# itxtx/normalizing-flows-study

Hardware: AMD Instinct MI355X
Metric: log_prob samples/sec/GPU + test-NLL match; RealNVP d=2 and MAF d=63 (higher is better)
Workload: dtype fp32

## Files before the change

normalizing-flows-study_amd/csrc/nfx_made.hip:

```cpp
#include "nfx_made_kernel.h"
#include "nfx_made_wide_kernel.h"
#include <atomic>
#include <cstdlib>

#include "nfx_made_seqs_kernel.h"
#include "nfx_pack.h"

namespace nfx {

__global__ void made_pack_kernel(NfxMlpRaw net, int d, int H, float* packed) {
    const int HT = (H + 31) / 32;
    const MadeLayout L = made_layout(d, HT);
    const int Hp = L.Hp, G1 = 4 * L.NKC;
    for (int i = blockIdx.x * blockDim.x + threadIdx.x; i < L.total; i += gridDim.x * blockDim.x) {
        if (i >= L.s_deg) continue;
        float v = 0.f;
        if (i < L.b1) {
            int t = i - L.w1, rr = t & 3, lane = (t >> 2) & 63, g = (t >> 8) % G1, ht = (t >> 8) / G1;
            int row = 32 * ht + (lane & 31), col = 2 * (4 * g + rr) + (lane >> 5);
            v = (row < H && col < d) ? mlp_weight(net, 0, d, row, col) : 0.f;
        } else if (i < L.w2) {
            int row = acc_vec_row(i - L.b1);
            v = row < H ? mlp_bias(net, 0, row) : 0.f;
        } else if (i < L.b2 || (i >= L.w3 && i < L.b3)) {
            const int layer = i < L.b2 ? 1 : 2;
            const ATileElem e = a_tile_elem(i - (layer == 1 ? L.w2 : L.w3));
            int row = 32 * (e.tile / HT) + e.row, col = 32 * (e.tile % HT) + e.k;
            v = (row < H && col < H) ? mlp_weight(net, layer, H, row, col) : 0.f;
        } else if (i < L.w3 || (i >= L.b3 && i < L.w4)) {
            const int layer = i < L.w3 ? 1 : 2;
            int row = acc_vec_row(i - (layer == 1 ? L.b2 : L.b3));
            v = row < H ? mlp_bias(net, layer, row) : 0.f;
        } else if (i < L.b4) {
            const ATileElem e = a_tile_elem(i - L.w4);
            int jw = e.tile / HT, which = jw & 1, j = jw >> 1;
            int orow = 32 * j + e.row, col = 32 * (e.tile % HT) + e.k;
            v = (orow < d && col < H) ? mlp_weight(net, 3, H, which * d + orow, col) : 0.f;
        } else if (i < L.par_total) {
            int t = i - L.b4, jw = t >> 5, which = jw & 1, j = jw >> 1;
            int orow = 32 * j + acc_vec_row(t & 31);
            v = orow < d ? mlp_bias(net, 3, which * d + orow) : 0.f;
        } else if (i < L.s_b1) {
            int t = i - L.s_w1t, ii = t / Hp, a = t % Hp;
            v = (ii < d && a < H) ? mlp_weight(net, 0, d, a, ii) : 0.f;
        } else if (i < L.s_w2) {
            int a = i - L.s_b1;
            v = a < H ? mlp_bias(net, 0, a) : 0.f;
        } else if (i < L.s_b2 || (i >= L.s_w3 && i < L.s_b3)) {
            const int layer = i < L.s_b2 ? 1 : 2;
            int t = i - (layer == 1 ? L.s_w2 : L.s_w3), a = t / Hp, b = t % Hp;
            v = (a < H && b < H) ? mlp_weight(net, layer, H, a, b) : 0.f;
        } else if (i < L.s_w3 || (i >= L.s_b3 && i < L.s_w4)) {
            const int layer = i < L.s_w3 ? 1 : 2;
            int a = i - (layer == 1 ? L.s_b2 : L.s_b3);
            v = a < H ? mlp_bias(net, layer, a) : 0.f;
        } else if (i < L.s_b4) {
            int t = i - L.s_w4, row = t / Hp, a = t % Hp;
            v = (row < 2 * d && a < H) ? mlp_weight(net, 3, H, row, a) : 0.f;
        } else if (i < L.s_deg) {
            int row = i - L.s_b4;
            v = row < 2 * d ? mlp_bias(net, 3, row) : 0.f;
        }
        packed[i] = v;
    }
}

constexpr int kLiveThreads = 1024;

__global__ __launch_bounds__(kLiveThreads) void made_live_kernel(NfxMlpRaw net, int d, int H, float* packed) {
    const int HT = (H + 31) / 32;
    const MadeLayout L = made_layout(d, HT);
    {
        __shared__ int deg[256];
        const int Hp = L.Hp;
        for (int a0 = 0; a0 < Hp; a0 += kLiveThreads / 16) {
            const int a = a0 + (threadIdx.x >> 4), q = threadIdx.x & 15;
            int n = 0;
            if (a < H && net.mask[0]) {
                const float* row = net.mask[0] + (size_t)a * d;
#pragma unroll 4
                for (int j = q; j < d; j += 16) n += row[j] != 0.f ? 1 : 0;
            }
            n += __shfl_xor(n, 1);
            n += __shfl_xor(n, 2);
            n += __shfl_xor(n, 4);
            n += __shfl_xor(n, 8);
            if (q == 0 && a < Hp) deg[a] = a < H ? (net.mask[0] ? n - 1 : 0) : 1000000000;
        }
        __syncthreads();
        for (int a = threadIdx.x; a < Hp; a += kLiveThreads) {
            const int da = deg[a];
            int rank = 0;
            for (int b = 0; b < Hp; ++b) rank += (deg[b] < da || (deg[b] == da && b < a)) ? 1 : 0;
            packed[L.s_deg + a] = (float)da;
            packed[L.s_deg + Hp + rank] = (float)da;
            packed[L.s_deg + 2 * Hp + rank] = (float)a;
        }
    }
    int* nk = reinterpret_cast<int*>(packed);
    for (int i = threadIdx.x; i < 3 * HT + L.NJ; i += kLiveThreads) nk[L.nk1 + i] = 0;
    __shared__ double red[256];
    const int rows[4] = {H, H, H, 2 * d}, cols[4] = {d, H, H, H};
    const double tsafe = block_mlp_tsafe(net, 4, rows, cols, 1.0e37, red);
    if (threadIdx.x == 0) packed[L.tsafe] = (float)fmin(tsafe, 3.0e38);
}

__global__ __launch_bounds__(256) void made_extent_kernel(int d, int H, float* packed) {
    const int HT = (H + 31) / 32;
    const MadeLayout L = made_layout(d, HT);
    int* nk = reinterpret_cast<int*>(packed);
    const int n1 = HT * 4 * L.NKC, n23 = HT * HT * 4, n4 = L.NJ * 2 * HT * 4;
    const int lane = lane_id();
    for (int gi = blockIdx.x * 4 + (threadIdx.x >> 6); gi < n1 + 2 * n23 + n4; gi += gridDim.x * 4) {
        int off, word, ext;
        if (gi < n1) {
            const int ht = gi / (4 * L.NKC), g = gi % (4 * L.NKC);
            off = L.w1 + gi * 256;
            word = L.nk1 + ht;
            ext = g / 4 + 1;
        } else if (gi < n1 + 2 * n23) {
            const int t = (gi - n1) % n23, layer = (gi - n1) / n23;
            off = (layer == 0 ? L.w2 : L.w3) + t * 256;
            word = (layer == 0 ? L.nk2 : L.nk3) + t / (HT * 4);
            ext = (t % (HT * 4)) / 4 + 1;
        } else {
            const int t = gi - n1 - 2 * n23;
            off = L.w4 + t * 256;
            word = L.nk4 + t / (2 * HT * 4);
            ext = (t % (HT * 4)) / 4 + 1;
        }
        const f32x4 v = *reinterpret_cast<const f32x4*>(packed + off + 4 * lane);
        const bool nzl = v[0] != 0.f || v[1] != 0.f || v[2] != 0.f || v[3] != 0.f;
        if (__ballot(nzl) != 0 && lane == 0) atomicMax(&nk[word], ext);
    }
}

template <int HT>
made_seqs_kernel_t made_seqs_pick_ht(int variant, bool logp) {
    if (variant == NFX_MAF_FORWARD) return made_seqs_kernel<HT, NFX_MAF_FORWARD, false>;
    return logp ? made_seqs_kernel<HT, NFX_IAF_INVERSE, true> : made_seqs_kernel<HT, NFX_IAF_INVERSE, false>;
}
template made_seqs_kernel_t made_seqs_pick_ht<1>(int, bool);
template made_seqs_kernel_t made_seqs_pick_ht<2>(int, bool);

template <int HT, int VAR>
static made_seq_kernel_t seq_var() {
    return made_seq_kernel<HT, VAR>;
}

template <int HT>
made_seq_kernel_t made_seq_pick_ht(int variant) {
    return variant == NFX_MAF_FORWARD ? seq_var<HT, NFX_MAF_FORWARD>() : seq_var<HT, NFX_IAF_INVERSE>();
}
template made_seq_kernel_t made_seq_pick_ht<1>(int);
template made_seq_kernel_t made_seq_pick_ht<2>(int);
template made_seq_kernel_t made_seq_pick_ht<3>(int);
template made_seq_kernel_t made_seq_pick_ht<4>(int);

static made_par_kernel_t pick_par(int HT, bool wlds, int variant) {
    return pick_range<1, 4>(HT, [=](auto HT_) { return made_pick_ht<HT_()>(wlds, variant); });
}

static made_par_kernel_t pick_tile(int HT, bool wlds, int variant, bool logp) {
    return pick_range<1, 4>(HT, [=](auto HT_) { return made_tile_pick_ht<HT_()>(wlds, variant, logp); });
}

static made_seq_kernel_t pick_seq(int HT, int variant) {
    return pick_range<1, 4>(HT, [=](auto HT_) { return made_seq_pick_ht<HT_()>(variant); });
}

int made_big_launch(const float* packed, const float* in, float* out, float* log_det, int64_t B, int d, int H,
                    int variant, int accumulate, hipStream_t s);

constexpr size_t kLdsBytes = 160 * 1024;
constexpr int kTileMaxD = 64;

}

using namespace nfx;

extern "C" size_t nfx_made_packed_floats(int d, int H) {
    if (d <= 0 || H <= 0) return 0;
    return (size_t)made_layout(d, (H + 31) / 32).total;
}

namespace nfx {
int made_pack_seqp(int d, int H, float* packed, hipStream_t s);
static int made_pack_seq(int d, int H, float* packed, hipStream_t s) {
    const int HT = (H + 31) / 32;
    if (HT > 2) return NFX_OK;
    if (HT == 1) made_seqs_image_kernel<1><<<64, 256, 0, s>>>(packed, d, H);
    else made_seqs_image_kernel<2><<<64, 256, 0, s>>>(packed, d, H);
    int rc = check_launch("made_seqs_image_kernel");
    if (rc) return rc;
    if (HT == 1) made_seqs_chunk_kernel<1><<<1, 64, 0, s>>>(packed, d, H);
    else made_seqs_chunk_kernel<2><<<1, 64, 0, s>>>(packed, d, H);
    rc = check_launch("made_seqs_chunk_kernel");
    if (rc) return rc;
    return made_pack_seqp(d, H, packed, s);
}
}

extern "C" int nfx_made_pack_parallel(const NfxMlpRaw* net, int d, int H, float* packed, void* stream) {
    if (!net || !packed) return set_error(NFX_EINVAL, "made_pack: null pointer");
    if (d <= 0 || d > 4096 || H <= 0 || H > 256)
        return set_error(NFX_EUNSUPPORTED, "made_pack: d=%d H=%d outside d<=4096, H<=256", d, H);
    if (net->n_layers != 4) return set_error(NFX_EINVAL, "made_pack: MADE has 4 masked layers (got %d)", net->n_layers);
    for (int l = 0; l < 4; ++l)
        if (!net->w[l]) return set_error(NFX_EINVAL, "made_pack: layer %d weight is null", l);
    const int total = (int)nfx_made_packed_floats(d, H);
    int blocks = (total + 255) / 256;
    if (blocks > 2048) blocks = 2048;
    made_pack_kernel<<<blocks, 256, 0, (hipStream_t)stream>>>(*net, d, H, packed);
    int rc = check_launch("made_pack_kernel");
    if (rc) return rc;
    made_live_kernel<<<1, kLiveThreads, 0, (hipStream_t)stream>>>(*net, d, H, packed);
    rc = check_launch("made_live_kernel");
    if (rc) return rc;
    {
        const int HT = (H + 31) / 32;
        const MadeLayout L = made_layout(d, HT);
        const int groups = HT * 4 * L.NKC + 2 * HT * HT * 4 + L.NJ * 2 * HT * 4;
        made_extent_kernel<<<(groups + 3) / 4, 256, 0, (hipStream_t)stream>>>(d, H, packed);
    }
    return check_launch("made_extent_kernel");
}

extern "C" int nfx_made_pack_sequential(int d, int H, float* packed, void* stream) {
    if (!packed) return set_error(NFX_EINVAL, "made_pack_sequential: null pointer");
    if (d <= 0 || d > 4096 || H <= 0 || H > 256)
        return set_error(NFX_EUNSUPPORTED, "made_pack_sequential: d=%d H=%d outside d<=4096, H<=256", d, H);
    return made_pack_seq(d, H, packed, (hipStream_t)stream);
}

extern "C" int nfx_made_pack(const NfxMlpRaw* net, int d, int H, float* packed, void* stream) {
    const int rc = nfx_made_pack_parallel(net, d, H, packed, stream);
    if (rc) return rc;
    return made_pack_seq(d, H, packed, (hipStream_t)stream);
}

namespace nfx {
int made_seqw_launch(const float* packed, const float* in, float* out, float* log_det, int64_t B, int d, int H,
                     int variant, int accumulate, float* logp, double* partials, double* sums, bool fused,
                     int* grid_out, hipStream_t s);
int made_seqp_launch(const float* packed, const float* in, float* out, float* log_det, int64_t B, int d, int H,
                     int variant, int accumulate, float* logp, double* partials, double* sums, bool fused,
                     hipStream_t s);
}

static std::atomic<int>& made_seq_policy() {
    static std::atomic<int> v{[] {
        const char* e = getenv("NFX_MADE_SEQ_POLICY");
        return e ? atoi(e) : NFX_MADE_SEQ_AUTO;
    }()};
    return v;
}

namespace nfx {
int made_seq_policy_get() { return made_seq_policy().load(std::memory_order_relaxed); }
}

static bool tile_path(int d, int HT, int variant) {
    return (variant == NFX_MAF_INVERSE || variant == NFX_IAF_FORWARD) && d > 0 && d <= kTileMaxD && HT >= 1 && HT <= 4;
}

struct TileConfig {
    int nw;
    bool wlds;
    size_t lds;
};
static TileConfig tile_config(const MadeLayout& L, int64_t ntiles, bool fused) {
    int nw = 8;
    if (!fused && ntiles < 4 * (int64_t)num_cus()) nw = (int)((ntiles + num_cus() - 1) / num_cus());
    const size_t wbytes = (size_t)L.par_total * sizeof(float);
    const size_t tiles = nw * 32 * (size_t)kTileStride * sizeof(float);
    const bool wlds = nw == 8 && wbytes + tiles <= kLdsBytes;
    return {nw, wlds, (wlds ? wbytes : 0) + tiles};
}

static int made_launch(const float* packed, const float* in, float* out, float* log_det, int64_t B,
                       int d, int H, int variant, int accumulate, float* logp, double* sums,
                       void* workspace, hipStream_t s) {
    const bool fused = sums != nullptr;
    if (B < 0 || d <= 0 || H <= 0) return set_error(NFX_EINVAL, "made_affine: bad shape");
    if (d > 4096 || H > 256) return set_error(NFX_EUNSUPPORTED, "made_affine: d=%d H=%d outside d<=4096, H<=256", d, H);
    if (variant < NFX_MAF_INVERSE || variant > NFX_IAF_INVERSE)
        return set_error(NFX_EINVAL, "made_affine: unknown variant %d", variant);
    const int HT = (H + 31) / 32;
    if (HT > 4) {
        if (fused) return set_error(NFX_EUNSUPPORTED, "made_affine_logprob: no fused log_prob for H=%d > 128", H);
        if (B == 0) return NFX_OK;
        if (!packed || !in || !out || !log_det) return set_error(NFX_EINVAL, "made_affine: null pointer");
        if (in == out) return set_error(NFX_EINVAL, "made_affine: in and out must not alias");
        return made_big_launch(packed, in, out, log_det, B, d, H, variant, accumulate, s);
    }
    const MadeLayout L = made_layout(d, HT);
    const bool parallel = variant == NFX_MAF_INVERSE || variant == NFX_IAF_FORWARD;
    const size_t wide_lds_bytes = (size_t)wide_lds(L, HT).total * sizeof(float);
    const bool wide = parallel && d > kTileMaxD && HT <= 2 && wide_lds_bytes <= kLdsBytes;
    const bool seqs = (variant == NFX_MAF_FORWARD || variant == NFX_IAF_INVERSE) && HT <= 2;
    if (fused && !((variant == NFX_MAF_INVERSE && (d <= kTileMaxD || wide)) || (variant == NFX_IAF_INVERSE && seqs)))
        return set_error(NFX_EUNSUPPORTED,
                         "made_affine_logprob: fused log_prob needs MAF inverse with d <= %d or H <= 64, "
                         "or IAF inverse with H <= 64", kTileMaxD);
    if (fused && B > 0 && (!logp || !workspace)) return set_error(NFX_EINVAL, "made_affine_logprob: null logp/workspace");
    if (B == 0) return fused ? gauss_finish(reinterpret_cast<double*>(workspace), 0, sums, 0, s) : NFX_OK;
    if (!packed || !in || !out || !log_det) return set_error(NFX_EINVAL, "made_affine: null pointer");
    if (in == out) return set_error(NFX_EINVAL, "made_affine: in and out must not alias");
    double* partials = reinterpret_cast<double*>(workspace);
    if (wide) {
        const int64_t nchunks = (B + 63) / 64;
        const int nw = nchunks < (int64_t)kWideWaves * num_cus() ? 4 : kWideWaves;
        const size_t lds_nw = (size_t)wide_lds(L, HT, nw).total * sizeof(float);
        made_par_kernel_t k = HT == 1 ? made_wide_pick_ht<1>(variant, fused, nw) : made_wide_pick_ht<2>(variant, fused, nw);
        int rc = prepare_lds((const void*)k, lds_nw);
        if (rc) return rc;
        int grid = resident_grid((const void*)k, 64 * nw, lds_nw, (nchunks + nw - 1) / nw);
        if (grid > kMaxPartials) grid = kMaxPartials;
        k<<<grid, 64 * nw, lds_nw, s>>>(packed, in, out, log_det, B, d, accumulate, nchunks, logp, partials,
                                        sums, gauss_const(d));
        return check_launch("made_wide_kernel");
    }
    if (tile_path(d, HT, variant)) {
        const int64_t ntiles = (B + 31) / 32;
        const TileConfig c = tile_config(L, ntiles, fused);
        made_par_kernel_t k = pick_tile(HT, c.wlds, variant, fused);
        if (!k) return set_error(NFX_EUNSUPPORTED, "made_affine: no kernel for H=%d", H);
        int rc = prepare_lds((const void*)k, c.lds);
        if (rc) return rc;
        int grid = resident_grid((const void*)k, 64 * c.nw, c.lds, (ntiles + c.nw - 1) / c.nw);
        if (grid > kMaxPartials) grid = kMaxPartials;
        k<<<grid, 64 * c.nw, c.lds, s>>>(packed, in, out, log_det, B, d, accumulate, ntiles, logp, partials, sums,
                                         gauss_const(d));
        return check_launch("made_tile_kernel");
    }
    if (variant == NFX_MAF_INVERSE || variant == NFX_IAF_FORWARD) {
        const size_t wbytes = (size_t)L.par_total * sizeof(float);
        const size_t stage8 = 8 * (size_t)kStageFloats * sizeof(float);
        const bool wlds = wbytes + stage8 <= kLdsBytes;
        made_par_kernel_t k = pick_par(HT, wlds, variant);
        if (!k) return set_error(NFX_EUNSUPPORTED, "made_affine: no kernel for H=%d", H);
        const int threads = wlds ? 512 : 256;
        const size_t lds = wlds ? wbytes + stage8 : 4 * (size_t)kStageFloats * sizeof(float);
        int rc = prepare_lds((const void*)k, lds);
        if (rc) return rc;
        const int64_t nchunks = (B + 63) / 64;
        const int nw = threads / 64;
        const int grid = resident_grid((const void*)k, threads, lds, (nchunks + nw - 1) / nw);
        k<<<grid, threads, lds, s>>>(packed, in, out, log_det, B, d, accumulate, nchunks, nullptr, nullptr, nullptr,
                                     0.f);
        return check_launch("made_parallel_kernel");
    }
    const int seq_pol = made_seq_policy().load(std::memory_order_relaxed);
    const bool push_auto = seq_pol == NFX_MADE_SEQ_AUTO && d > 32 && B <= 4096 * (int64_t)num_cus() / 256;
    if (seqs && (seq_pol == NFX_MADE_SEQ_PUSH || push_auto) && L.ps > 0)
        return made_seqp_launch(packed, in, out, log_det, B, d, H, variant, accumulate, logp, partials, sums, fused, s);
    if (seqs && (seq_pol == NFX_MADE_SEQ_PUSH || seq_pol == NFX_MADE_SEQ_WAVE || (seq_pol == NFX_MADE_SEQ_AUTO && B <= 2048 * (int64_t)num_cus() / 256))) {
        int grid = 0;
        return made_seqw_launch(packed, in, out, log_det, B, d, H, variant, accumulate, logp, partials, sums, fused,
                                &grid, s);
    }
    if (seqs) {
        made_seqs_kernel_t k = HT == 1 ? made_seqs_pick_ht<1>(variant, fused) : made_seqs_pick_ht<2>(variant, fused);
        const size_t lds = (size_t)seqs_lds(L.Hp).total * sizeof(float);
        int rc = prepare_lds((const void*)k, lds);
        if (rc) return rc;
        const int threads = kSeqsThreads;
        int grid = resident_grid((const void*)k, threads, lds, (B + 4 * kSeqsWaves - 1) / (4 * kSeqsWaves));
        if (grid > kMaxPartials) grid = kMaxPartials;
        k<<<grid, threads, lds, s>>>(packed, in, out, log_det, B, d, H, accumulate, logp, partials, sums,
                                     gauss_const(d));
        return check_launch("made_seqs_kernel");
    }
    made_seq_kernel_t k = pick_seq(HT, variant);
    if (!k) return set_error(NFX_EUNSUPPORTED, "made_affine: no sequential kernel for H=%d", H);
    const size_t lds = 2 * 64 * (size_t)(L.Hp + 4) * sizeof(float);
    int rc = prepare_lds((const void*)k, lds);
    if (rc) return rc;
    const int64_t grid = (B + 63) / 64;
    k<<<(unsigned)grid, 64, lds, s>>>(packed, in, out, log_det, B, d, H, accumulate);
    return check_launch("made_seq_kernel");
}

extern "C" int nfx_made_seq_policy(int policy) {
    if (policy < 0) return made_seq_policy().load();
    if (policy > NFX_MADE_SEQ_PUSH) return set_error(NFX_EINVAL, "made_seq_policy: unknown policy %d", policy);
    return made_seq_policy().exchange(policy);
}

extern "C" int nfx_made_affine(const float* packed, const float* in, float* out, float* log_det,
                               int64_t B, int d, int H, int variant, int accumulate, void* stream) {
    return made_launch(packed, in, out, log_det, B, d, H, variant, accumulate, nullptr, nullptr, nullptr,
                       (hipStream_t)stream);
}

extern "C" int nfx_made_affine_logprob(const float* packed, const float* in, float* out, float* log_det,
                                       float* logp, double* sums, void* workspace, int64_t B, int d,
                                       int H, int variant, int accumulate, void* stream) {
    if (!sums) return set_error(NFX_EINVAL, "made_affine_logprob: null sums");
    return made_launch(packed, in, out, log_det, B, d, H, variant, accumulate, logp, sums, workspace,
                       (hipStream_t)stream);
}

extern "C" int nfx_made_sample_supported(int d, int H, int variant) {
    return (H > 0 && tile_path(d, (H + 31) / 32, variant) && variant == NFX_IAF_FORWARD) ? 1 : 0;
}

extern "C" int nfx_made_affine_sample(const float* packed, uint64_t seed, uint64_t* rng_state, float* z, float* x,
                                      float* log_det, int64_t B, int d, int H, void* stream) {
    if (B < 0 || d <= 0 || H <= 0) return set_error(NFX_EINVAL, "made_affine_sample: bad shape");
    if (!nfx_made_sample_supported(d, H, NFX_IAF_FORWARD))
        return set_error(NFX_EUNSUPPORTED, "made_affine_sample: d=%d H=%d outside the tile kernel (d <= %d, H <= 128)",
                         d, H, kTileMaxD);
    if (B == 0) return NFX_OK;
    if (!packed || !rng_state || !z || !x || !log_det) return set_error(NFX_EINVAL, "made_affine_sample: null pointer");
    if (z == x) return set_error(NFX_EINVAL, "made_affine_sample: z and x must not alias");
    const int HT = (H + 31) / 32;
    const MadeLayout L = made_layout(d, HT);
    const int64_t ntiles = (B + 31) / 32;
    const TileConfig c = tile_config(L, ntiles, false);
    made_sample_kernel_t k =
        pick_range<1, 4>(HT, [=](auto HT_) { return made_tile_sample_pick_ht<HT_()>(c.wlds); });
    int rc = prepare_lds((const void*)k, c.lds);
    if (rc) return rc;
    int grid = resident_grid((const void*)k, 64 * c.nw, c.lds, (ntiles + c.nw - 1) / c.nw);
    if (grid > kMaxPartials) grid = kMaxPartials;
    k<<<grid, 64 * c.nw, c.lds, (hipStream_t)stream>>>(packed, nullptr, x, log_det, B, d, 0, ntiles, nullptr, nullptr,
                                                       nullptr, 0.f, MadeDraw{seed, rng_state, z});
    return check_launch("made_tile_kernel");
}
```

normalizing-flows-study_amd/csrc/nfx_made_kernel.h:

```cpp
#pragma once
#include "nfx_common.h"
#include "nfx_rng.h"

namespace nfx {

struct MadeLayout {
    int d, HT, Hp, NKC, NJ;
    int w1, b1, w2, b2, w3, b3, w4, b4;
    int par_total;
    int s_w1t, s_b1, s_w2, s_b2, s_w3, s_b3, s_w4, s_b4, s_deg;
    int nk1, nk2, nk3, nk4, tsafe;
    int t4, t3, t2, t1;
    int rimg;
    int sw1, sw4, sb4;
    int ctab;
    int ps, pw4, pw1, pb4, pw23, ptb, ptab;
    int total;
};

__host__ __device__ constexpr int made_up4(int v) { return (v + 3) & ~3; }

__host__ __device__ constexpr int seqs_w4_stride(int Hp) { return 2 * Hp + 4; }
constexpr int kSeqsPadRows = 64;
__host__ __device__ constexpr int seqs_max_chunks(int d, int Hp) { return d / 8 + 2 * Hp + 8; }
constexpr int kSeqpMaxS = 16;
__host__ __device__ constexpr int seqp_slots(int d, int HT) {
    return (HT <= 2 && d <= 64 * kSeqpMaxS) ? (d + 63) / 64 : 0;
}
__host__ __device__ constexpr int seqp_max_chunks(int d, int Hp) { return (d + 63) / 64 + 3 * Hp + 4; }

__host__ __device__ constexpr MadeLayout made_layout(int d, int HT) {
    MadeLayout L{};
    L.d = d;
    L.HT = HT;
    L.Hp = 32 * HT;
    L.NKC = (d + 31) / 32;
    L.NJ = (d + 31) / 32;
    int o = 0;
    L.w1 = o; o += HT * 4 * L.NKC * 256;
    L.b1 = o; o += HT * 32;
    L.w2 = o; o += HT * HT * 1024;
    L.b2 = o; o += HT * 32;
    L.w3 = o; o += HT * HT * 1024;
    L.b3 = o; o += HT * 32;
    L.w4 = o; o += L.NJ * 2 * HT * 1024;
    L.b4 = o; o += L.NJ * 2 * 32;
    L.par_total = o;
    L.s_w1t = o; o += made_up4(d * L.Hp);
    L.s_b1 = o; o += L.Hp;
    L.s_w2 = o; o += L.Hp * L.Hp;
    L.s_b2 = o; o += L.Hp;
    L.s_w3 = o; o += L.Hp * L.Hp;
    L.s_b3 = o; o += L.Hp;
    L.s_w4 = o; o += made_up4(2 * d * L.Hp);
    L.s_b4 = o; o += made_up4(2 * d);
    L.s_deg = o; o += 3 * L.Hp;
    L.nk1 = o; o += HT;
    L.nk2 = o; o += HT;
    L.nk3 = o; o += HT;
    L.nk4 = o; o += L.NJ;
    L.tsafe = o; o += 1;
    o = made_up4(o);
    L.t4 = o; o += HT * 2 * L.NJ * 1024;
    L.t3 = o; o += HT * HT * 1024;
    L.t2 = o; o += HT * HT * 1024;
    L.t1 = o; o += L.NKC * HT * 1024;
    L.rimg = o; o += HT <= 2 ? 2 * L.Hp * L.Hp + 5 * L.Hp : 0;
    o = made_up4(o);
    const int rows = HT <= 2 ? d + kSeqsPadRows : 0;
    L.sw1 = o; o += made_up4(rows * L.Hp);
    L.sw4 = o; o += made_up4(rows * seqs_w4_stride(L.Hp));
    L.sb4 = o; o += made_up4(2 * rows);
    L.ctab = o; o += HT <= 2 ? 8 * seqs_max_chunks(d, L.Hp) : 0;
    const int PS = seqp_slots(d, HT);
    L.ps = PS;
    L.pw4 = o; o += L.Hp * ((PS + 1) / 2) * 256;
    L.pw1 = o; o += L.Hp * ((PS + 3) / 4) * 256;
    L.pb4 = o; o += PS * 128;
    L.pw23 = o; o += PS ? 2 * L.Hp * L.Hp : 0;
    L.ptb = o; o += PS ? 4 * L.Hp : 0;
    L.ptab = o; o += PS ? 16 * seqp_max_chunks(d, L.Hp) : 0;
    L.total = o;
    return L;
}

constexpr int kStageStride = 33;
constexpr int kTileStride = 65;
constexpr int kStageFloats = 64 * kStageStride;

template <int VAR>
__device__ __forceinline__ float made_affine(float xv, float mu, float al, float& acc) {
#pragma clang fp contract(off)
    if constexpr (VAR == NFX_MAF_INVERSE) {
        const float a = tclamp(al, -3.f, 3.f);
        acc = acc + a;
        const float z = (xv - mu) * exp_fast(-a);
        return nonfinite(z) ? 0.f : z;
    } else {
        const float a = tclamp(al, -2.f, 2.f);
        const float m = tclamp(mu, -10.f, 10.f);
        acc = acc + a;
        const float y = xv * exp_fast(a) + m;
        return nonfinite(y) ? xv : y;
    }
}

__device__ __forceinline__ void stage_in(const float* __restrict__ in, int64_t base, int d, int64_t B,
                                         int dim0, float* st) {
    const int lane = lane_id();
#pragma unroll 8
    for (int i = 0; i < 32; ++i) {
        const int idx = i * 64 + lane;
        const int s = idx >> 5, dd = idx & 31;
        const int64_t row = base + s;
        const int dim = dim0 + dd;
        st[s * kStageStride + dd] = (row < B && dim < d) ? in[row * d + dim] : 0.f;
    }
}

__device__ __forceinline__ void stage_out(float* __restrict__ out, int64_t base, int d, int64_t B,
                                          int dim0, const float* st) {
    const int lane = lane_id();
#pragma unroll 8
    for (int i = 0; i < 32; ++i) {
        const int idx = i * 64 + lane;
        const int s = idx >> 5, dd = idx & 31;
        const int64_t row = base + s;
        const int dim = dim0 + dd;
        if (row < B && dim < d) out[row * d + dim] = st[s * kStageStride + dd];
    }
}


template <int HT>
__device__ __forceinline__ void made_hidden(const float* __restrict__ W, int woff, int boff,
                                            const f32x16 (&hin)[HT][2], f32x16 (&hout)[HT][2]) {
    const int lane = lane_id(), h = lane >> 5;
#pragma unroll
    for (int hto = 0; hto < HT; ++hto) {
        f32x16 a0, a1;
        load_bias16_x2(W + boff + hto * 32, h, a0, a1);
#pragma unroll
        for (int kt = 0; kt < HT; ++kt) {
#pragma unroll
            for (int rq = 0; rq < 4; ++rq) {
                const f32x4 w = *reinterpret_cast<const f32x4*>(W + woff + (a_quad(a_tile(hto, kt, HT), rq) * 64 + lane) * 4);
#pragma unroll
                for (int rr = 0; rr < 4; ++rr) {
                    a0 = mfma32(w[rr], hin[kt][0][4 * rq + rr], a0);
                    a1 = mfma32(w[rr], hin[kt][1][4 * rq + rr], a1);
                }
            }
        }
#pragma unroll
        for (int r = 0; r < 16; ++r) {
            a0[r] = trelu(a0[r]);
            a1[r] = trelu(a1[r]);
        }
        hout[hto][0] = a0;
        hout[hto][1] = a1;
    }
}

template <int HT, bool WLDS, int VAR>
__global__ __launch_bounds__(WLDS ? 512 : 256) void made_parallel_kernel(
    const float* __restrict__ packed, const float* __restrict__ in, float* __restrict__ out,
    float* __restrict__ logdet, int64_t B, int d, int accumulate, int64_t nchunks,
    float* __restrict__ , double* __restrict__ , double* __restrict__ ,
    float ) {
    constexpr int NWAVE = WLDS ? 8 : 4;
    const MadeLayout L = made_layout(d, HT);
    extern __shared__ f32x4 lds4[];
    float* lds = reinterpret_cast<float*>(lds4);
    const int wave = threadIdx.x >> 6;
    float* stg;
    if constexpr (WLDS) {
        const f32x4* src = reinterpret_cast<const f32x4*>(packed);
        for (int i = threadIdx.x; i < L.par_total / 4; i += NWAVE * 64) lds4[i] = src[i];
        stg = lds + L.par_total + wave * kStageFloats;
        __syncthreads();
    } else {
        stg = lds + wave * kStageFloats;
    }
    const int lane = lane_id(), h = lane >> 5, col = lane & 31;
    const int64_t nwaves = (int64_t)gridDim.x * NWAVE;

    for (int64_t c = (int64_t)blockIdx.x * NWAVE + wave; c < nchunks; c += nwaves) {
        const int64_t base = c * 64;
        const float* W = (WLDS ? lds : packed) + opaque_zero();

        f32x16 h1[HT][2];
#pragma unroll
        for (int ht = 0; ht < HT; ++ht) load_bias16_x2(W + L.b1 + ht * 32, h, h1[ht][0], h1[ht][1]);
        for (int kc = 0; kc < L.NKC; ++kc) {
            stage_in(in, base, d, B, 32 * kc, stg);
            wave_lds_sync();
#pragma unroll
            for (int g = 0; g < 4; ++g) {
                f32x4 w[HT];
#pragma unroll
                for (int ht = 0; ht < HT; ++ht)
                    w[ht] = *reinterpret_cast<const f32x4*>(W + L.w1 + ((ht * 4 * L.NKC + kc * 4 + g) * 64 + lane) * 4);
#pragma unroll
                for (int rr = 0; rr < 4; ++rr) {
                    const int k = 8 * g + 2 * rr + h;
                    const float b0 = stg[col * kStageStride + k];
                    const float b1 = stg[(32 + col) * kStageStride + k];
#pragma unroll
                    for (int ht = 0; ht < HT; ++ht) {
                        h1[ht][0] = mfma32(w[ht][rr], b0, h1[ht][0]);
                        h1[ht][1] = mfma32(w[ht][rr], b1, h1[ht][1]);
                    }
                }
            }
            wave_lds_sync();
        }
#pragma unroll
        for (int ht = 0; ht < HT; ++ht) {
#pragma unroll
            for (int r = 0; r < 16; ++r) {
                h1[ht][0][r] = trelu(h1[ht][0][r]);
                h1[ht][1][r] = trelu(h1[ht][1][r]);
            }
        }
        f32x16 h2[HT][2];
        made_hidden<HT>(W, L.w2, L.b2, h1, h2);
        made_hidden<HT>(W, L.w3, L.b3, h2, h1);

        float acc0 = 0.f, acc1 = 0.f;
        for (int j = 0; j < L.NJ; ++j) {
            f32x16 mu0, mu1, al0, al1;
            load_bias16_x2(W + L.b4 + (j * 2 + 0) * 32, h, mu0, mu1);
            load_bias16_x2(W + L.b4 + (j * 2 + 1) * 32, h, al0, al1);
#pragma unroll
// ... 478 lines not shown
```

normalizing-flows-study_amd/csrc/nfx_tile.h:

```cpp
#pragma once

#include <hip/hip_runtime.h>

namespace nfx {

__host__ __device__ constexpr int crow(int r, int h) { return (r & 3) + 8 * (r >> 2) + 4 * h; }
__host__ __device__ constexpr int creg(int row) { return (row & 3) + 4 * (row >> 3); }
__host__ __device__ constexpr int chalf(int row) { return (row >> 2) & 1; }

struct RowCol {
    int row, col;
};

struct ATileElem {
    int tile, row, k;
};
__host__ __device__ constexpr ATileElem a_tile_elem(int t) {
    const int rr = t & 3, lane = (t >> 2) & 63, rq = (t >> 8) & 3;
    return {t >> 10, lane & 31, crow(4 * rq + rr, lane >> 5)};
}
__host__ __device__ constexpr int a_tile(int ot, int kt, int NK) { return ot * NK + kt; }
__host__ __device__ constexpr int a_quad(int tile, int rq) { return tile * 4 + rq; }

__host__ __device__ constexpr RowCol a1_elem(int t, int KS1) {
    const int lane = t & 63, ks = (t >> 6) % KS1, ht = (t >> 6) / KS1;
    return {32 * ht + (lane & 31), 2 * ks + (lane >> 5)};
}

__host__ __device__ constexpr int acc_vec_row(int t) { return 32 * (t >> 5) + crow(t & 15, (t >> 4) & 1); }

__host__ __device__ constexpr RowCol acc_dump_elem(int t) { return {crow(t >> 6, (t >> 5) & 1), t & 31}; }
__host__ __device__ constexpr int acc_dump_index(int row, int col) {
    return creg(row) * 64 + chalf(row) * 32 + col;
}
__host__ __device__ constexpr RowCol lane_dump_elem(int t) { return {crow(t & 15, (t >> 9) & 1), (t >> 4) & 31}; }

namespace tile_check {
constexpr bool crow_round_trips() {
    for (int row = 0; row < 32; ++row)
        if (crow(creg(row), chalf(row)) != row) return false;
    for (int r = 0; r < 16; ++r)
        for (int h = 0; h < 2; ++h)
            if (creg(crow(r, h)) != r || chalf(crow(r, h)) != h) return false;
    return true;
}
constexpr bool a_tile_visits_all() {
    bool seen[32 * 32] = {};
    for (int t = 0; t < 1024; ++t) {
        const ATileElem e = a_tile_elem(t);
        if (e.tile != 0 || e.row < 0 || e.row > 31 || e.k < 0 || e.k > 31 || seen[e.row * 32 + e.k]) return false;
        seen[e.row * 32 + e.k] = true;
    }
    return true;
}
constexpr bool a_tile_encode_inverts() {
    for (int t = 0; t < 3 * 1024; ++t) {
        const ATileElem e = a_tile_elem(t);
        const int r = creg(e.k), lane = e.row + 32 * chalf(e.k);
        if ((a_quad(e.tile, r >> 2) * 64 + lane) * 4 + (r & 3) != t) return false;
    }
    return true;
}
constexpr bool dumps_round_trip() {
    bool seen[32 * 32] = {};
    for (int t = 0; t < 1024; ++t) {
        const RowCol e = acc_dump_elem(t), l = lane_dump_elem(t);
        if (acc_dump_index(e.row, e.col) != t) return false;
        if (l.row < 0 || l.row > 31 || l.col < 0 || l.col > 31 || seen[l.row * 32 + l.col]) return false;
        seen[l.row * 32 + l.col] = true;
    }
    return true;
}
static_assert(crow_round_trips(), "creg/chalf invert crow for all 32 rows");
static_assert(a_tile_visits_all(), "A-operand decode is a bijection onto the tile");
static_assert(a_tile_encode_inverts(), "A-operand encode inverts the decode");
static_assert(dumps_round_trip(), "accumulator dump orders are bijections");
static_assert(acc_vec_row(32 + 16 + 5) == 32 + crow(5, 1), "accumulator-order vector");
}

}
```

Measured before the change: 1.666 billion.

## Add split-bf16 MFMA tile kernel for MADE inverse with fp32 fallback

Adds a new MADE tile kernel for MAF inverse with d<=64 and H<=64. It replaces the fp32 MFMA chain with a three-way bf16 split of weights and activations, using six bf16 MFMAs per block to emulate fp32 accuracy. A new pack kernel prepares the split weights: two pieces live in LDS, the third is read from global memory. It also computes a safe input bound, and any tile whose inputs exceed that bound falls back to the fp32 MFMA path. The kernel prefetches the next tile's inputs and runs by default for large batches, controlled by NFX_MADE_SPLIT. The cost is more pack-time work, more complexity and a small accuracy risk on the NLL match.

```diff
diff --git a/normalizing-flows-study_amd/csrc/nfx_made.hip b/normalizing-flows-study_amd/csrc/nfx_made.hip
--- a/normalizing-flows-study_amd/csrc/nfx_made.hip
+++ b/normalizing-flows-study_amd/csrc/nfx_made.hip
@@ -5,6 +5,12 @@
 
 #include "nfx_made_seqs_kernel.h"
 #include "nfx_pack.h"
+
+namespace nfx {
+int made_split_pack(float* packed, int d, int H, hipStream_t s);
+template <int HT>
+made_par_kernel_t made_tile_split_pick_ht(bool logp);
+}
 
 namespace nfx {
 
@@ -223,7 +229,9 @@
         const int groups = HT * 4 * L.NKC + 2 * HT * HT * 4 + L.NJ * 2 * HT * 4;
         made_extent_kernel<<<(groups + 3) / 4, 256, 0, (hipStream_t)stream>>>(d, H, packed);
     }
-    return check_launch("made_extent_kernel");
+    rc = check_launch("made_extent_kernel");
+    if (rc) return rc;
+    return made_split_pack(packed, d, H, (hipStream_t)stream);
 }
 
 extern "C" int nfx_made_pack_sequential(int d, int H, float* packed, void* stream) {
@@ -276,6 +284,21 @@
     const size_t tiles = nw * 32 * (size_t)kTileStride * sizeof(float);
     const bool wlds = nw == 8 && wbytes + tiles <= kLdsBytes;
     return {nw, wlds, (wlds ? wbytes : 0) + tiles};
+}
+
+struct SplitConfig {
+    int nw;
+    size_t lds;
+};
+static SplitConfig split_config(int d, int HT, int variant, int64_t ntiles) {
+    if (variant != NFX_MAF_INVERSE || !made_has_split(d, HT)) return {0, 0};
+    const char* e = getenv("NFX_MADE_SPLIT");
+    const int mode = e ? atoi(e) : 1;
+    if (mode == 0 || (mode != 2 && ntiles < 8 * (int64_t)num_cus())) return {0, 0};
+    const int nw = 8;
+    const size_t lds = ((size_t)made_split(d, HT).stage + nw * 32 * (size_t)kTileStride) * sizeof(float);
+    if (lds + 1024 > kLdsBytes) return {0, 0};
+    return {nw, lds};
 }
 
 static int made_launch(const float* packed, const float* in, float* out, float* log_det, int64_t B,
@@ -323,6 +346,17 @@
     }
     if (tile_path(d, HT, variant)) {
         const int64_t ntiles = (B + 31) / 32;
+        const SplitConfig sc = split_config(d, HT, variant, ntiles);
+        if (sc.nw) {
+            made_par_kernel_t k = HT == 1 ? made_tile_split_pick_ht<1>(fused) : made_tile_split_pick_ht<2>(fused);
+            int rc = prepare_lds((const void*)k, sc.lds);
+            if (rc) return rc;
+            int grid = resident_grid((const void*)k, 64 * sc.nw, sc.lds, (ntiles + sc.nw - 1) / sc.nw);
+            if (grid > kMaxPartials) grid = kMaxPartials;
+            k<<<grid, 64 * sc.nw, sc.lds, s>>>(packed, in, out, log_det, B, d, accumulate, ntiles, logp, partials, sums,
+                                               gauss_const(d));
+            return check_launch("made_tile_split_kernel");
+        }
         const TileConfig c = tile_config(L, ntiles, fused);
         made_par_kernel_t k = pick_tile(HT, c.wlds, variant, fused);
         if (!k) return set_error(NFX_EUNSUPPORTED, "made_affine: no kernel for H=%d", H);
diff --git a/normalizing-flows-study_amd/csrc/nfx_made_kernel.h b/normalizing-flows-study_amd/csrc/nfx_made_kernel.h
--- a/normalizing-flows-study_amd/csrc/nfx_made_kernel.h
+++ b/normalizing-flows-study_amd/csrc/nfx_made_kernel.h
@@ -15,6 +15,7 @@
     int sw1, sw4, sb4;
     int ctab;
     int ps, pw4, pw1, pb4, pw23, ptb, ptab;
+    int sp;
     int total;
 };
 
@@ -28,6 +29,37 @@
     return (HT <= 2 && d <= 64 * kSeqpMaxS) ? (d + 63) / 64 : 0;
 }
 __host__ __device__ constexpr int seqp_max_chunks(int d, int Hp) { return (d + 63) / 64 + 3 * Hp + 4; }
+
+struct MadeSplit {
+    int w1, w2, w3, w4;
+    int b1, b2, b3, b4;
+    int stage;
+    int v1, v2, v3, v4;
+    int ok, total;
+};
+__host__ __device__ constexpr bool made_has_split(int d, int HT) { return d <= 64 && HT <= 2; }
+__host__ __device__ constexpr MadeSplit made_split(int d, int HT) {
+    MadeSplit S{};
+    const int NKC = (d + 31) / 32, NJ = NKC;
+    const int n1 = HT * 2 * NKC, n23 = HT * 2 * HT, n4 = 2 * NJ * 2 * HT;
+    int o = 0;
+    S.w1 = o; o += n1 * 512;
+    S.w2 = o; o += n23 * 512;
+    S.w3 = o; o += n23 * 512;
+    S.w4 = o; o += n4 * 512;
+    S.b1 = o; o += HT * 32;
+    S.b2 = o; o += HT * 32;
+    S.b3 = o; o += HT * 32;
+    S.b4 = o; o += NJ * 2 * 32;
+    S.stage = o;
+    S.v1 = o; o += n1 * 256;
+    S.v2 = o; o += n23 * 256;
+    S.v3 = o; o += n23 * 256;
+    S.v4 = o; o += n4 * 256;
+    S.ok = o;
+    S.total = o + 4;
+    return S;
+}
 
 __host__ __device__ constexpr MadeLayout made_layout(int d, int HT) {
     MadeLayout L{};
@@ -80,6 +112,8 @@
     L.pw23 = o; o += PS ? 2 * L.Hp * L.Hp : 0;
     L.ptb = o; o += PS ? 4 * L.Hp : 0;
     L.ptab = o; o += PS ? 16 * seqp_max_chunks(d, L.Hp) : 0;
+    o = made_up4(o);
+    L.sp = o; o += made_has_split(d, HT) ? made_split(d, HT).total : 0;
     L.total = o;
     return L;
 }
diff --git a/normalizing-flows-study_amd/csrc/nfx_made_split.hip b/normalizing-flows-study_amd/csrc/nfx_made_split.hip
--- /dev/null
+++ b/normalizing-flows-study_amd/csrc/nfx_made_split.hip
@@ -0,0 +1,113 @@
+#include "nfx_made_split_kernel.h"
+
+namespace nfx {
+
+namespace {
+__device__ __forceinline__ int par_weight(const MadeLayout& L, int l, int row, int k) {
+    if (l == 1) return L.w1 + made_a1_index(row >> 5, 4 * L.NKC, row & 31, k);
+    const int base = l == 2 ? L.w2 : l == 3 ? L.w3 : L.w4;
+    return base + a_tile_index(a_tile(row >> 5, k >> 5, L.HT), row & 31, k & 31);
+}
+__device__ __forceinline__ int par_bias(const MadeLayout& L, int l, int row) {
+    return (l == 1 ? L.b1 : l == 2 ? L.b2 : l == 3 ? L.b3 : L.b4) + acc_vec_index(row);
+}
+}
+
+__global__ __launch_bounds__(1024) void made_split_pack_kernel(float* packed, int d, int H) {
+    const int HT = (H + 31) / 32;
+    const MadeLayout L = made_layout(d, HT);
+    const MadeSplit S = made_split(d, HT);
+    float* out = packed + L.sp;
+    const int rows[5] = {0, L.Hp, L.Hp, L.Hp, 64 * L.NJ}, cols[5] = {0, 32 * L.NKC, L.Hp, L.Hp, L.Hp};
+    __shared__ int w_bad;
+    __shared__ float rowsum[4][128], babs[4][128];
+    if (threadIdx.x == 0) w_bad = 0;
+    __syncthreads();
+    bool bad = false;
+    for (int i = threadIdx.x; i < S.ok; i += blockDim.x) {
+        uint32_t v;
+        if (i >= S.b1 && i < S.stage) {
+            const int src = i < S.b2 ? L.b1 + (i - S.b1) : i < S.b3 ? L.b2 + (i - S.b2)
+                          : i < S.b4 ? L.b3 + (i - S.b3) : L.b4 + (i - S.b4);
+            v = __float_as_uint(packed[src]);
+        } else {
+            const bool third = i >= S.stage;
+            const int l = third ? (i < S.v2 ? 1 : i < S.v3 ? 2 : i < S.v4 ? 3 : 4)
+                                : (i < S.w2 ? 1 : i < S.w3 ? 2 : i < S.w4 ? 3 : 4);
+            const int nkb = l == 1 ? 2 * L.NKC : 2 * HT;
+            const int base = third ? (l == 1 ? S.v1 : l == 2 ? S.v2 : l == 3 ? S.v3 : S.v4)
+                                   : (l == 1 ? S.w1 : l == 2 ? S.w2 : l == 3 ? S.w3 : S.w4);
+            SplitDword e = split_dword(i - base, third ? 1 : 2);
+            if (third) e.piece = 2;
+            const int ot = e.block / nkb, kb = e.block % nkb, hh = e.lane >> 5;
+            uint32_t half[2];
+            for (int c = 0; c < 2; ++c) {
+                const int k = l == 1 ? split_col(kb, hh, 2 * e.q + c)
+                                     : 32 * (kb >> 1) + crow(split_reg(kb, 2 * e.q + c), hh);
+                const float w = packed[par_weight(L, l, 32 * ot + (e.lane & 31), k)];
+                if (!(fabsf(w) <= 1e6f)) bad = true;
+                const uint32_t u0 = __builtin_bit_cast(uint16_t, (__bf16)w);
+                const float r1 = w - __uint_as_float(u0 << 16);
+                const uint32_t u1 = __builtin_bit_cast(uint16_t, (__bf16)r1);
+                const uint32_t u2 = __builtin_bit_cast(uint16_t, (__bf16)(r1 - __uint_as_float(u1 << 16)));
+                half[c] = e.piece == 0 ? u0 : e.piece == 1 ? u1 : u2;
+            }
+            v = half[0] | (half[1] << 16);
+        }
+        out[i] = __uint_as_float(v);
+    }
+    if (bad) atomicOr(&w_bad, 1);
+    if (threadIdx.x < 4 * 128) {
+        const int l = 1 + threadIdx.x / 128, row = threadIdx.x % 128;
+        float sum = 0.f, b = 0.f;
+        if (row < rows[l]) {
+            for (int k = 0; k < cols[l]; ++k) sum += fabsf(packed[par_weight(L, l, row, k)]);
+            b = fabsf(packed[par_bias(L, l, row)]);
+        }
+        rowsum[l - 1][row] = sum;
+        babs[l - 1][row] = b;
+    }
+    __syncthreads();
+    if (threadIdx.x == 0) {
+        double alpha = 1.0, beta = 0.0, ssafe = fmin((double)packed[L.tsafe], 1e30);
+        double n[4];
+        for (int l = 0; l < 4; ++l) {
+            double nmax = 0.0, cmax = 0.0;
+            for (int r = 0; r < 128; ++r) {
+                const double s = rowsum[l][r], b = babs[l][r];
+                nmax = (s > nmax || s != s) ? s : nmax;
+                cmax = (b > cmax || b != b) ? b : cmax;
+            }
+            n[l] = nmax;
+            alpha = nmax * alpha;
+            beta = nmax * beta + cmax;
+            if (!(beta < 1e30) || !(alpha < 1e300)) ssafe = 0.0;
+            else if (alpha > 0.0) ssafe = fmin(ssafe, (1e30 - beta) / alpha);
+        }
+        double cut = 0.0, prod = 1.0;
+        for (int l = 3; l >= 0; --l) {
+            prod *= n[l];
+            cut += prod;
+        }
+        const bool lost = !(0x1p-133 * cut < 0x1p-24);
+        out[S.ok] = (w_bad || lost || !(ssafe > 0.0)) ? 0.f : 1.f;
+        out[S.ok + 1] = ssafe > 0.0 ? (float)ssafe : 0.f;
+        out[S.ok + 2] = 0.f;
+        out[S.ok + 3] = 0.f;
+    }
+}
+
+int made_split_pack(float* packed, int d, int H, hipStream_t s) {
+    if (!made_has_split(d, (H + 31) / 32)) return NFX_OK;
+    made_split_pack_kernel<<<1, 1024, 0, s>>>(packed, d, H);
+    return check_launch("made_split_pack_kernel");
+}
+
+template <int HT>
+made_par_kernel_t made_tile_split_pick_ht(bool logp) {
+    return logp ? made_tile_split_kernel<HT, true> : made_tile_split_kernel<HT, false>;
+}
+template made_par_kernel_t made_tile_split_pick_ht<1>(bool);
+template made_par_kernel_t made_tile_split_pick_ht<2>(bool);
+
+}
diff --git a/normalizing-flows-study_amd/csrc/nfx_made_split_kernel.h b/normalizing-flows-study_amd/csrc/nfx_made_split_kernel.h
--- /dev/null
+++ b/normalizing-flows-study_amd/csrc/nfx_made_split_kernel.h
@@ -0,0 +1,276 @@
+#pragma once
+#include "nfx_affine_kernel.h"
+#include "nfx_made_kernel.h"
+
+namespace nfx {
+
+constexpr int kSplitTileWaves = 8;
+
+constexpr int kMadeTermW[6] = {1, 0, 1, 0, 2, 0}, kMadeTermX[6] = {1, 2, 0, 1, 0, 0};
+
+__device__ __forceinline__ void load_w01(const float* __restrict__ Wp, int blk, u32x4 (&w)[2]) {
+    const u32x4* wq = reinterpret_cast<const u32x4*>(Wp) + lane_id();
+    w[0] = wq[split_quad(blk, 0, 2) * 64];
+    w[1] = wq[split_quad(blk, 1, 2) * 64];
+}
+
+__device__ __forceinline__ void split_mac(const u32x4 (&w01)[2], u32x4 w2, const u32x4 (&xp)[3], f32x16& hi,
+                                          f32x16& lo) {
+    const u32x4 w[3] = {w01[0], w01[1], w2};
+    static_for<6>([&](auto t) {
+        constexpr int T = decltype(t)::value;
+        if constexpr (T == 5) {
+            hi = mfma_bf16(w[kMadeTermW[T]], xp[kMadeTermX[T]], hi);
+        } else {
+            lo = mfma_bf16(w[kMadeTermW[T]], xp[kMadeTermX[T]], lo);
+        }
+    });
+}
+
+template <int NKB, class Third>
+__device__ __forceinline__ void split_chain(const float* __restrict__ Wp, int ot, int nkbs, int nkb,
+                                            const u32x4 (&xin)[NKB][3], Third&& third, f32x16& hi, f32x16& lo) {
+    __builtin_amdgcn_s_setprio(2);
+#pragma unroll
+    for (int kb = 0; kb < NKB; ++kb) {
+        if (kb < nkb) {
+            u32x4 w[2];
+            load_w01(Wp, split_blk(ot, kb, nkbs), w);
+            split_mac(w, third(kb), xin[kb], hi, lo);
+        }
+    }
+    __builtin_amdgcn_s_setprio(0);
+}
+
+template <int NKB>
+__device__ __forceinline__ void load_third(const float* __restrict__ Vg, int ot, int nkbs, int nkb,
+                                           u32x4 (&v)[NKB]) {
+    const u32x4* vq = reinterpret_cast<const u32x4*>(Vg) + lane_id();
+#pragma unroll
+    for (int kb = 0; kb < NKB; ++kb)
+        if (kb < nkb) v[kb] = vq[split_quad(split_blk(ot, kb, nkbs), 0, 1) * 64];
+}
+
+__device__ __forceinline__ f32x16 zero16() {
+    return f32x16{0.f, 0.f, 0.f, 0.f, 0.f, 0.f, 0.f, 0.f, 0.f, 0.f, 0.f, 0.f, 0.f, 0.f, 0.f, 0.f};
+}
+
+template <int HT, int NKB>
+__device__ __forceinline__ void split_hidden(const float* __restrict__ Wp, const float* __restrict__ Vg,
+                                             const float* __restrict__ bias, int nkbs, const u32x4 (&xin)[NKB][3],
+                                             const int (&nkb)[HT], u32x4 (&xout)[2 * HT][3]) {
+    const int h = lane_id() >> 5;
+    u32x4 v[HT][NKB];
+#pragma unroll
+    for (int hto = 0; hto < HT; ++hto) load_third<NKB>(Vg, hto, nkbs, nkb[hto], v[hto]);
+#pragma unroll
+    for (int hto = 0; hto < HT; ++hto) {
+        f32x16 hi = load_bias16(bias + hto * 32, h), lo = zero16();
+        split_chain<NKB>(Wp, hto, nkbs, nkb[hto], xin, [&](int kb) { return v[hto][kb]; }, hi, lo);
+        f32x16 a;
+#pragma unroll
+        for (int r = 0; r < 16; ++r) a[r] = trelu(hi[r] + lo[r]);
+        split_block(a, 0, xout[2 * hto]);
+        split_block(a, 1, xout[2 * hto + 1]);
+    }
+}
+
+template <int HT>
+__device__ __forceinline__ f32x16 split_out_tile(const float* __restrict__ Wp, const float* __restrict__ Vg,
+                                                 const float* __restrict__ bias, int ot,
+                                                 const u32x4 (&xin)[2 * HT][3], int nkb) {
+    const u32x4* vq = reinterpret_cast<const u32x4*>(Vg) + lane_id();
+    u32x4 v = {}, vn = {};
+    if (0 < nkb) v = vq[split_quad(split_blk(ot, 0, 2 * HT), 0, 1) * 64];
+    f32x16 hi = load_bias16(bias + ot * 32, lane_id() >> 5), lo = zero16();
+    split_chain<2 * HT>(Wp, ot, 2 * HT, nkb, xin, [&](int kb) {
+        const u32x4 cur = v;
+        if (kb + 1 < 2 * HT && kb + 1 < nkb) vn = vq[split_quad(split_blk(ot, kb + 1, 2 * HT), 0, 1) * 64];
+        v = vn;
+        return cur;
+    }, hi, lo);
+    f32x16 o;
+#pragma unroll
+    for (int r = 0; r < 16; ++r) o[r] = hi[r] + lo[r];
+    return o;
+}
+
+template <int HT, bool LOGP>
+__global__ __launch_bounds__(64 * kSplitTileWaves) void made_tile_split_kernel(
+    const float* __restrict__ packed, const float* __restrict__ in, float* __restrict__ out,
+    float* __restrict__ logdet, int64_t B, int d, int accumulate, int64_t ntiles, float* __restrict__ logp,
+    double* __restrict__ partials, double* __restrict__ sums, float cgauss) {
+    constexpr int NW = kSplitTileWaves;
+    static_assert(HT <= 2, "the split tail exists for H <= 64");
+    constexpr int VAR = NFX_MAF_INVERSE;
+    constexpr int NKB1 = 4;
+    const MadeLayout L = made_layout(d, HT);
+    const MadeSplit SL = made_split(d, HT);
+    constexpr int S = kTileStride;
+    extern __shared__ f32x4 lds4[];
+    float* lds = reinterpret_cast<float*>(lds4);
+    const int wave = __builtin_amdgcn_readfirstlane(threadIdx.x >> 6);
+    {
+        const f32x4* src = reinterpret_cast<const f32x4*>(packed + L.sp);
+        for (int i = threadIdx.x; i < SL.stage / 4; i += 64 * NW) lds4[i] = src[i];
+    }
+    float* xt = lds + SL.stage + wave * 32 * S;
+    __syncthreads();
+    const int lane = lane_id(), h = lane >> 5, col = lane & 31;
+    const int64_t nwaves = (int64_t)gridDim.x * NW;
+    const int voff = lane < d ? lane * 4 : (1 << 30);
+    const int rowb = d * 4;
+    const int* nkp = reinterpret_cast<const int*>(packed);
+    int nkb1[HT], nkb2[HT], nkb3[HT];
+    int nkb1max = 0;
+#pragma unroll
+    for (int i = 0; i < HT; ++i) {
+        nkb1[i] = 2 * nkp[L.nk1 + i];
+        nkb2[i] = 2 * nkp[L.nk2 + i];
+        nkb3[i] = 2 * nkp[L.nk3 + i];
+        nkb1max = nkb1[i] > nkb1max ? nkb1[i] : nkb1max;
+    }
+    const float ssafe = packed[L.sp + SL.ok] != 0.f ? packed[L.sp + SL.ok + 1] : -1.f;
+
+    int64_t t = (int64_t)blockIdx.x * NW + wave;
+    double lpacc = 0.0;
+    float pf[32];
+    float ldpf = 0.f;
+    {
+        if (accumulate && t < ntiles && lane < 32 && t * 32 + col < B) ldpf = logdet[t * 32 + col];
+        const int64_t rows = t < ntiles ? (B - t * 32 < 32 ? B - t * 32 : 32) : 0;
+        const auto rs = __builtin_amdgcn_make_buffer_rsrc(const_cast<float*>(in) + (t < ntiles ? t * 32 * d : 0), 0,
+                                                          (int)(rows * rowb), 0x00020000);
+#pragma unroll
+        for (int r = 0; r < 32; ++r)
+            pf[r] = __uint_as_float(__builtin_amdgcn_raw_buffer_load_b32(rs, voff, r * rowb, 0));
+    }
+    for (; t < ntiles; t += nwaves) {
+        const int64_t base = t * 32;
+        const int rows = (int)(B - base < 32 ? B - base : 32);
+        const float* Ws = lds + opaque_zero();
+        const float* Wg = packed + opaque_zero();
+        const float* Vg = packed + L.sp + opaque_zero();
+        float xmax = 0.f;
+#pragma unroll
+        for (int r = 0; r < 32; ++r) {
+            xt[r * S + lane] = pf[r];
+            xmax = tmax(xmax, fabsf(pf[r]));
+        }
+        const bool fb = __builtin_amdgcn_ballot_w64(!(xmax <= ssafe)) != 0;
+        wave_lds_sync();
+
+        auto finish = [&](auto&& pair) __attribute__((always_inline)) {
+                const float ldin = ldpf;
+            {
+                const int64_t tn = t + nwaves;
+                ldpf = (accumulate && tn < ntiles && lane < 32 && tn * 32 + col < B) ? logdet[tn * 32 + col] : 0.f;
+                const int64_t rn = tn < ntiles ? (B - tn * 32 < 32 ? B - tn * 32 : 32) : 0;
+                const auto rs = __builtin_amdgcn_make_buffer_rsrc(const_cast<float*>(in) + (tn < ntiles ? tn * 32 * d : 0), 0,
+                                                                  (int)(rn * rowb), 0x00020000);
+#pragma unroll
+                for (int r = 0; r < 32; ++r)
+                    pf[r] = __uint_as_float(__builtin_amdgcn_raw_buffer_load_b32(rs, voff, r * rowb, 0));
+            }
+
+            float acc = 0.f;
+            for (int j = 0; j < L.NJ; ++j) {
+                f32x16 mu, al;
+                pair(j, mu, al);
+#pragma unroll
+                for (int r = 0; r < 16; ++r) {
+                    float* p = xt + col * S + 32 * j + crow(r, h);
+                    *p = made_affine<VAR>(*p, mu[r], al[r], acc);
+                }
+            }
+            const float ssum = halves_sum(acc, acc);
+            wave_lds_sync();
+            float zsq = 0.f;
+            if constexpr (LOGP) {
+                if (lane < 32) {
+                    for (int jd = 0; jd < d; ++jd) {
+                        const float v = xt[col * S + jd];
+                        zsq = (jd == 0) ? gauss_sq0(v) : gauss_sq(zsq, v);
+                    }
+                }
+            }
+            {
+                const auto rs = __builtin_amdgcn_make_buffer_rsrc(out + base * d, 0, rows * rowb, 0x00020000);
+#pragma unroll
+                for (int r = 0; r < 32; ++r)
+                    __builtin_amdgcn_raw_buffer_store_b32(__float_as_uint(xt[r * S + lane]), rs, voff, r * rowb, 0);
+            }
+            if (lane < 32 && col < rows) {
+                float ldv = -ssum;
+                if (nonfinite(ldv)) ldv = 0.f;
+                ldv = tclamp(ldv, -100.f, 100.f);
+                const int64_t so = base + col;
+                const float ldt = accumulate ? ldin + ldv : ldv;
+                logdet[so] = ldt;
+                if constexpr (LOGP) {
+                    const float lp = gauss_lp(zsq, cgauss, ldt);
+                    logp[so] = lp;
+                    lpacc += (double)lp;
+                }
+            }
+        };
+        if (fb) {
+            f32x16 h1[HT];
+#pragma unroll
+            for (int ht = 0; ht < HT; ++ht) {
+                f32x16 a = load_bias16(Wg + L.b1 + ht * 32, h);
+                for (int kc = 0; kc < L.NKC; ++kc) {
+#pragma unroll
+                    for (int g = 0; g < 4; ++g) {
+                        const f32x4 w = *reinterpret_cast<const f32x4*>(
+                            Wg + L.w1 + ((ht * 4 * L.NKC + kc * 4 + g) * 64 + lane) * 4);
+#pragma unroll
+                        for (int rr = 0; rr < 4; ++rr)
+                            a = mfma32(w[rr], xt[col * S + 32 * kc + 8 * g + 2 * rr + h], a);
+                    }
+                }
+#pragma unroll
+                for (int r = 0; r < 16; ++r) a[r] = trelu(a[r]);
+                h1[ht] = a;
+            }
+            f32x16 h2[HT];
+            made_hidden1<HT>(Wg, L.w2, L.b2, h1, h2);
+            made_hidden1<HT>(Wg, L.w3, L.b3, h2, h1);
+            finish([&](int j, f32x16& mu, f32x16& al) { out_pair<HT, HT>(Wg, L, j, h1, mu, al); });
+        } else {
+            u32x4 x1[NKB1][3];
+#pragma unroll
+            for (int kb = 0; kb < NKB1; ++kb) {
+                if (kb < nkb1max) {
+#pragma unroll
+                    for (int q = 0; q < 4; ++q) {
+                        uint32_t l0, l1, l2, g0, g1, g2;
+                        split3(xt[col * S + split_col(kb, h, 2 * q)], l0, l1, l2);
+                        split3(xt[col * S + split_col(kb, h, 2 * q + 1)], g0, g1, g2);
+                        x1[kb][0][q] = pack_bf16(l0, g0);
+                        x1[kb][1][q] = pack_bf16(l1, g1);
+                        x1[kb][2][q] = pack_bf16(l2, g2);
+                    }
+                }
+            }
+            u32x4 x2[2 * HT][3], x3[2 * HT][3], xp[2 * HT][3];
+            split_hidden<HT, NKB1>(Ws + SL.w1, Vg + SL.v1, Ws + SL.b1, 2 * L.NKC, x1, nkb1, x2);
+            split_hidden<HT, 2 * HT>(Ws + SL.w2, Vg + SL.v2, Ws + SL.b2, 2 * HT, x2, nkb2, x3);
+            split_hidden<HT, 2 * HT>(Ws + SL.w3, Vg + SL.v3, Ws + SL.b3, 2 * HT, x3, nkb3, xp);
+            finish([&](int j, f32x16& mu, f32x16& al) {
+                mu = split_out_tile<HT>(Ws + SL.w4, Vg + SL.v4, Ws + SL.b4, j * 2 + 0, xp, 2 * nkp[L.nk4 + j]);
+                al = split_out_tile<HT>(Ws + SL.w4, Vg + SL.v4, Ws + SL.b4, j * 2 + 1, xp, 2 * nkp[L.nk4 + j]);
+            });
+        }
+
+        wave_lds_sync();
+    }
+    if constexpr (LOGP) {
+        logp_commit<64 * NW>(lpacc, partials, sums, B);
+    }
+}
+
+template <int HT>
+made_par_kernel_t made_tile_split_pick_ht(bool logp);
+
+}
diff --git a/normalizing-flows-study_amd/csrc/nfx_tile.h b/normalizing-flows-study_amd/csrc/nfx_tile.h
--- a/normalizing-flows-study_amd/csrc/nfx_tile.h
+++ b/normalizing-flows-study_amd/csrc/nfx_tile.h
@@ -35,7 +35,64 @@
 }
 __host__ __device__ constexpr RowCol lane_dump_elem(int t) { return {crow(t & 15, (t >> 9) & 1), (t >> 4) & 31}; }
 
+struct SplitDword {
+    int block, piece, lane, q;
+};
+__host__ __device__ constexpr SplitDword split_dword(int t, int NP) {
+    return {(t >> 8) / NP, (t >> 8) % NP, (t >> 2) & 63, t & 3};
+}
+__host__ __device__ constexpr int split_blk(int ot, int kb, int NKB) { return ot * NKB + kb; }
+__host__ __device__ constexpr int split_quad(int block, int p, int NP) { return block * NP + p; }
+__host__ __device__ constexpr int split_reg(int kb, int e) { return 8 * (kb & 1) + e; }
+__host__ __device__ constexpr int split_col(int kb, int h, int e) { return 16 * kb + 8 * h + e; }
+
+__host__ __device__ constexpr int made_a1_index(int ht, int G1, int row, int col) {
+    return ((ht * G1 + (col >> 3)) * 64 + row + 32 * (col & 1)) * 4 + ((col >> 1) & 3);
+}
+__host__ __device__ constexpr int a_tile_index(int tile, int row, int k) {
+    return (a_quad(tile, creg(k) >> 2) * 64 + row + 32 * chalf(k)) * 4 + (creg(k) & 3);
+}
+__host__ __device__ constexpr int acc_vec_index(int row) {
+    return 32 * (row >> 5) + 16 * chalf(row & 31) + creg(row & 31);
+}
+
 namespace tile_check {
+constexpr bool split_dword_visits_all() {
+    for (int NP = 1; NP <= 3; ++NP) {
+        bool seen[2 * 768] = {};
+        for (int t = 0; t < 2 * 256 * NP; ++t) {
+            const SplitDword e = split_dword(t, NP);
+            const int i = (split_quad(e.block, e.piece, NP) * 64 + e.lane) * 4 + e.q;
+            if (e.block != t / (256 * NP) || e.piece >= NP || i != t || seen[i]) return false;
+            seen[i] = true;
+        }
+    }
+    for (int kb = 0; kb < 4; ++kb) {
+        bool col[64] = {}, reg[64] = {};
+        for (int h = 0; h < 2; ++h)
+            for (int e = 0; e < 8; ++e) {
+                const int c = split_col(kb, h, e), r = 32 * (kb >> 1) + crow(split_reg(kb, e), h);
+                if (c < 16 * kb || c >= 16 * kb + 16 || col[c] || reg[r]) return false;
+                col[c] = reg[r] = true;
+            }
+    }
+    return true;
+}
+constexpr bool made_indices_invert() {
+    for (int t = 0; t < 2 * 1024; ++t) {
+        const ATileElem e = a_tile_elem(t);
+        if (a_tile_index(e.tile, e.row, e.k) != t) return false;
+    }
+    for (int t = 0; t < 64; ++t)
+        if (acc_vec_index(acc_vec_row(t)) != t) return false;
+    for (int t = 0; t < 2 * 8 * 256; ++t) {
+        const int rr = t & 3, lane = (t >> 2) & 63, g = (t >> 8) % 8, ht = (t >> 8) / 8;
+        if (made_a1_index(ht, 8, lane & 31, 2 * (4 * g + rr) + (lane >> 5)) != t) return false;
+    }
+    return true;
+}
+static_assert(split_dword_visits_all(), "split block decode is a bijection; operand orders cover a k block");
+static_assert(made_indices_invert(), "A-tile, accumulator-vector and MADE layer-1 encodes invert their decodes");
 constexpr bool crow_round_trips() {
     for (int row = 0; row < 32; ++row)
         if (crow(creg(row), chalf(row)) != row) return false;
```

Measured after the change: 1.666 billion, median of 2. About the same (-0.0%).
